# idthanm/env_build

Hardware: AMD Instinct MI355X
Metric: env-steps/s (batched rollout) at N_env x N_veh; achieved HBM GB/s vs peak (higher is better)
Workload: dtype f32

## Files before the change

env_build_amd/csrc/eb_rollout.hip:

```cpp
#include <type_traits>

#include "eb_device.h"
#include "eb_kernels.h"

#pragma clang fp contract(off)

namespace eb {

typedef float f2u __attribute__((ext_vector_type(2), aligned(4)));
typedef float v2f __attribute__((ext_vector_type(2)));
EB_DEV v2f fma2(v2f a, v2f b, v2f c) { return __builtin_elementwise_fma(a, b, c); }

template <typename ST> struct Stored;
template <> struct Stored<float> {
    static EB_DEV f4u load4(const float* p) { return *reinterpret_cast<const f4u*>(p); }
    static EB_DEV float load1(const float* p) { return *p; }
    static EB_DEV void store4(float* p, f4u v) { *reinterpret_cast<f4u*>(p) = v; }
    static EB_DEV void store1(float* p, float v) { *p = v; }
    static EB_DEV float round(float v) { return v; }
    static EB_DEV void store4_wt(float* p, f4u v) { asm volatile("global_store_dwordx4 %0, %1, off sc1\n\ts_nop 1" :: "v"(p), "v"(v) : "memory"); }
    static EB_DEV void store1_wt(float* p, float v) { asm volatile("global_store_dword %0, %1, off sc1" :: "v"(p), "v"(v) : "memory"); }
};
typedef _Float16 h4u __attribute__((ext_vector_type(4), aligned(2)));
template <> struct Stored<_Float16> {
    static EB_DEV f4u load4(const _Float16* p) {
        const h4u h = *reinterpret_cast<const h4u*>(p);
        return f4u{(float)h.x, (float)h.y, (float)h.z, (float)h.w};
    }
    static EB_DEV float load1(const _Float16* p) { return (float)*p; }
    static EB_DEV void store4(_Float16* p, f4u v) {
        *reinterpret_cast<h4u*>(p) = h4u{(_Float16)v.x, (_Float16)v.y, (_Float16)v.z, (_Float16)v.w};
    }
    static EB_DEV void store1(_Float16* p, float v) { *p = (_Float16)v; }
    static EB_DEV float round(float v) { return (float)(_Float16)v; }
    static EB_DEV void store4_wt(_Float16* p, f4u v) {
        typedef unsigned u2v __attribute__((ext_vector_type(2)));
        const u2v bits = __builtin_bit_cast(u2v, h4u{(_Float16)v.x, (_Float16)v.y, (_Float16)v.z, (_Float16)v.w});
        asm volatile("global_store_dwordx2 %0, %1, off sc1" :: "v"(p), "v"(bits) : "memory");
    }
    static EB_DEV void store1_wt(_Float16* p, float v) {
        const unsigned bits = __builtin_bit_cast(unsigned short, (_Float16)v);
        asm volatile("global_store_short %0, %1, off sc1" :: "v"(p), "v"(bits) : "memory");
    }
};

EB_DEV void lds_barrier() { asm volatile("s_waitcnt lgkmcnt(0)\n\ts_barrier" ::: "memory"); }
typedef __attribute__((address_space(3))) int lds_int;
EB_DEV void lds_publish(int* flag, int value) {
    asm volatile("s_waitcnt lgkmcnt(0)" ::: "memory");
    *(volatile lds_int*)flag = value;
}
EB_DEV void lds_wait_until(int* flag, int value) {
    while (*(volatile lds_int*)flag != value) __builtin_amdgcn_s_sleep(2);
    asm volatile("" ::: "memory");
}

template <int CTRL, int ROW_MASK>
EB_DEV double dpp_f64(double v) {
    const unsigned long long b = __builtin_bit_cast(unsigned long long, v);
    const unsigned lo = (unsigned)__builtin_amdgcn_update_dpp(0, (int)(unsigned)b, CTRL, ROW_MASK, 0xf, false);
    const unsigned hi = (unsigned)__builtin_amdgcn_update_dpp(0, (int)(unsigned)(b >> 32), CTRL, ROW_MASK, 0xf, false);
    return __builtin_bit_cast(double, ((unsigned long long)hi << 32) | lo);
}
EB_DEV double wave_sum_f64(double v) {
    v += dpp_f64<0x111, 0xf>(v);
    v += dpp_f64<0x112, 0xf>(v);
    v += dpp_f64<0x114, 0xf>(v);
    v += dpp_f64<0x118, 0xf>(v);
    v += dpp_f64<0x142, 0xa>(v);
    v += dpp_f64<0x143, 0xc>(v);
    return v;
}
template <int CTRL, int ROW_MASK>
EB_DEV float dpp_max_f32(float v) {
    const float o = __builtin_bit_cast(float, __builtin_amdgcn_update_dpp(0, __builtin_bit_cast(int, v), CTRL, ROW_MASK, 0xf, false));
    return o > v ? o : v;
}
EB_DEV float wave_max_f32(float v) {
    v = dpp_max_f32<0x111, 0xf>(v);
    v = dpp_max_f32<0x112, 0xf>(v);
    v = dpp_max_f32<0x114, 0xf>(v);
    v = dpp_max_f32<0x118, 0xf>(v);
    v = dpp_max_f32<0x142, 0xa>(v);
    v = dpp_max_f32<0x143, 0xc>(v);
    return v;
}

EB_DEV void acc_record(double* recs, bool act, int lane, float v_r, float v_t, float v_p) {
    const double s_r = wave_sum_f64(act ? (double)v_r : 0.0);
    const double s_t = wave_sum_f64(act ? (double)v_t : 0.0);
    const double s_p = wave_sum_f64(act ? (double)v_p : 0.0);
    const unsigned long long any = __builtin_amdgcn_ballot_w64(act && v_p > 0.0f);
    if (lane == 63) {
        typedef double d2v __attribute__((ext_vector_type(2)));
        d2v* rec = reinterpret_cast<d2v*>(recs + (size_t)ACC_RECORD_DOUBLES * blockIdx.x);
        rec[0] = d2v{s_r, s_t};
        rec[1] = d2v{s_p, __builtin_bit_cast(double, any)};
    }
}

EB_DEV unsigned agent_load_u32(const unsigned* p) {
    unsigned v;
    asm volatile("global_load_dword %0, %1, off sc1\n\ts_waitcnt vmcnt(0)" : "=v"(v) : "v"(p) : "memory");
    return v;
}
EB_DEV unsigned long long agent_load_u64(const void* p) {
    unsigned long long v;
    asm volatile("global_load_dwordx2 %0, %1, off sc1\n\ts_waitcnt vmcnt(0)" : "=v"(v) : "v"(p) : "memory");
    return v;
}
EB_DEV void agent_store_u32(unsigned* p, unsigned v) { asm volatile("global_store_dword %0, %1, off sc1" :: "v"(p), "v"(v) : "memory"); }
EB_DEV void agent_add_u32(unsigned* p, unsigned v) { asm volatile("global_atomic_add %0, %1, off sc1" :: "v"(p), "v"(v) : "memory"); }

template <typename ST>
struct FusedHot {
    const ST* obs_in;
    ST* obs_out;
    int n_env, obs_dim, n_veh, envs_per_tile;
    unsigned nv_magic;
    int do_rewards;
    double* acc_rec;
    const unsigned char* turn;
    long long t_entry;
};
constexpr int HOT_REWARDS = 1, HOT_PRIO = 2;

template <typename ST>
EB_DEV int env_of_item(const FusedHot<ST>& H, int item) {
    return H.nv_magic ? (int)__umulhi((unsigned)item, H.nv_magic) : item;
}

#define EB_MARK(A, row, i) do { if ((A).trace && (threadIdx.x & 63) == 0) (A).trace[(size_t)(row) * 8 + (i)] = wall_clock64(); } while (0)
#define EB_MARK_PLACE(A, row) do { if ((A).trace && (threadIdx.x & 63) == 0) (A).trace[(size_t)(row) * 8 + 7] = \
    ((long long)__builtin_amdgcn_s_getreg((31 << 11) | 20) << 32) | (unsigned)__builtin_amdgcn_s_getreg((31 << 11) | 4); } while (0)

constexpr int QCAP = 160;
constexpr int TAPE_QCAP = 192;

template <int PRE = 3, bool COARSE = true>
EB_DEV int closest_cell_index(const FusedArgs& A, const float* xy10, const float* phi10, int p, int roff, float px, float py,
                              float& rx, float& ry, float& rphi) {
    const float* xy = xy10 + 2 * roff;
    const float* ph = phi10 + roff;
    const float fx = (px - A.gx0) * CELL_INV, fy = (py - A.gy0) * CELL_INV;
    unsigned c = 0xffffffffu;
    if (fx >= 0.0f && fx < (float)A.gnx && fy >= 0.0f && fy < (float)A.gny) c = A.cells[(p * A.gny + (int)fy) * A.gnx + (int)fx];
    if (c == 0xffffffffu) {
        int r_first = 0, r_last = 1 << 30;
        if constexpr (COARSE) {
            const PathTables& pt = *A.dt;
            int lo, hi, lo2, hi2;
            const int how = coarse_cell_ranges(pt, p, px, py, lo, hi, lo2, hi2);
            if (how == 1) return closest_in_ranges(xy, ph, lo, hi, lo2, hi2, px, py, rx, ry, rphi);
            if (how == 2) { r_first = lo; r_last = hi; }
        }
        const int n = p == 0 ? A.red_len[0] : p == 1 ? A.red_len[1] : A.red_len[2];
        const int bi = closest_reduced_index(reinterpret_cast<const float2*>(xy), A.rad_all + 32 * p, n, px, py, r_first, r_last);
        rx = xy[2 * bi]; ry = xy[2 * bi + 1]; rphi = ph[bi];
        return bi;
    }
    if (PRE > 0 && A.scan_one_trip) return closest_in_range<0>(xy, ph, (int)(c & 0xffffu), (int)(c >> 16), px, py, rx, ry, rphi);
    return closest_in_range<PRE>(xy, ph, (int)(c & 0xffffu), (int)(c >> 16), px, py, rx, ry, rphi);
}

template <int RW, int RPT>
struct FusedSmem {
    static constexpr int ITEMS = RW * 64 * RPT;
    float4 ego[64];
    unsigned char turn[64];
    unsigned long long mask[64];
    float2 pen[ITEMS];
    v2f qxy[RW][QCAP];
    v2f qsc[RW][QCAP];
    int qitem[RW][QCAP];
    int ego_ready;
    int waves_done;
};

template <int TASK, int RW, int RPT, typename ST>
EB_DEV void env_wave(const FusedHot<ST>& H, const FusedArgs& A, FusedSmem<RW, RPT>& S, int e0, int nE) {
    const int lane = threadIdx.x;
    const int D = H.obs_dim, NV = H.n_veh;
    const bool act = lane < nE;
    const int e = act ? lane : 0, ge = e0 + e;
    const ST* hin = H.obs_in + (size_t)ge * D;
    ST* hout = H.obs_out + (size_t)ge * D;

    const f4u h0 = Stored<ST>::load4(hin), h1 = Stored<ST>::load4(hin + 4);
    const float h8 = Stored<ST>::load1(hin + 8);
    const f2u araw = *reinterpret_cast<const f2u*>(A.actions + 2 * (size_t)ge);
    int p = A.path_id;
    if (A.training) {
        const int pr = A.ref_idx[ge];
        p = (pr >= 0 && pr < A.n_paths) ? pr : -1;
    }
    float sh_prev = 0.0f;
    if (A.shield_punish && !A.shield_first && act) sh_prev = A.shield_punish[ge];
    const int trow = blockIdx.x * (RW + 1);
    if (lane == 0) { S.ego_ready = 0; S.waves_done = 0; }
    lds_barrier();
    EB_MARK(A, trow, 0);
    EB_MARK_PLACE(A, trow);
    const bool do_rewards = (H.do_rewards & HOT_REWARDS) != 0;
    const float st[6] = {h0.x, h0.y, h0.z, h0.w, h1.x, h1.y};
    const float phi_rad = deg2rad(st[5]);
    float es, ec;
    sincos_det(phi_rad, es, ec);
    if (do_rewards) {
        S.ego[lane] = make_float4(st[3], st[4], es, ec);
        S.mask[lane] = 0ull;
        lds_publish(&S.ego_ready, 1);
        EB_MARK(A, trow, 1);
    }

    float steer, a_x;
    if (A.actions_raw) action_transform(araw.x, araw.y, steer, a_x);
    else { steer = araw.x; a_x = araw.y; }
    if (act && A.scaled_actions) *reinterpret_cast<f2u*>(A.scaled_actions + 2 * (size_t)ge) = f2u{steer, a_x};
    float rew = 0.0f;
    if (act && do_rewards) {
        const float punish_steer = -sq(steer), punish_a_x = -sq(a_x);
        const float punish_yaw_rate = -sq(st[2]);
        const float devi_y = -sq(h1.z);
        const float devi_phi = -sq(deg2rad(h1.w));
        const float devi_v = -sq(h8);
        rew = 0.05f * devi_v + 0.8f * devi_y + 30.0f * devi_phi + 0.02f * punish_yaw_rate +
              5.0f * punish_steer + 0.05f * punish_a_x;
        A.out5[ge] = rew;
    }
    float nx[6];
    f_xu_core(st, steer, a_x, TAU10, phi_rad, es, ec, nx);
    nx[0] = __builtin_fminf(__builtin_fmaxf(nx[0], 0.0f), 35.0f);
    float t0 = 0.0f, t1 = 0.0f, t2 = 0.0f;
    if (p >= 0) {
        const int roff = p == 0 ? A.red_off[0] : p == 1 ? A.red_off[1] : A.red_off[2];
        EB_MARK(A, trow, 2);
        float rx = 0.0f, ry = 0.0f, rphi = 0.0f;
        constexpr int SCAN_PRE = RW * RPT >= 32 ? 0 : 3;
        const int bi = closest_cell_index<SCAN_PRE>(A, A.xy10, A.phi10, p, roff, nx[3], nx[4], rx, ry, rphi);
        t0 = two2one<TASK>(nx[3], nx[4], rx, ry);
        if (A.trace) { asm volatile("" :: "v"(t0)); EB_MARK(A, trow, 3); }
        t1 = deal_with_phi_diff(nx[5] - rphi);
        t2 = nx[0] - EXP_V;
        if (A.n_future > 0 && act) {
            const PathTables& pt = *A.dt;
            const int len = pt.len[p];
            ST* otrk = hout + 9;
            int cur = bi * 10;
            for (int k = 0; k < A.n_future; ++k) {
                cur += 80;
                if (cur >= len - 2) cur = len - 2;
                const int fi = clamp_index(cur, len);
                Stored<ST>::store1(otrk + 3 * k, pt.x[p][fi] - nx[3]);
                Stored<ST>::store1(otrk + 3 * k + 1, pt.y[p][fi] - nx[4]);
                Stored<ST>::store1(otrk + 3 * k + 2, deal_with_phi_diff(nx[5] - pt.phi[p][fi]));
            }
        }
    } else if (A.n_future > 0 && act) {
        ST* otrk = hout + 9;
        for (int c = 0; c < 3 * A.n_future; ++c) Stored<ST>::store1(otrk + c, 0.0f);
    }
    if (act) {
        Stored<ST>::store4(hout, f4u{nx[0], nx[1], nx[2], nx[3]});
        Stored<ST>::store4(hout + 4, f4u{nx[4], nx[5], t0, t1});
        Stored<ST>::store1(hout + 8, t2);
    }
    EB_MARK(A, trow, 4);
    if (!do_rewards) return;
    float road_t = 0.0f, road_r = 0.0f;
    road_terms<TASK>(st[3] + LWS * ec, st[4] + LWS * es, road_t, road_r);
    road_terms<TASK>(st[3] - LWS * ec, st[4] - LWS * es, road_t, road_r);
    lds_wait_until(&S.waves_done, RW);
    EB_MARK(A, trow, 5);

    float pun_t = 0.0f, pun_r = 0.0f;
    if (act) {
        float a35 = 0.0f, a25 = 0.0f;
        unsigned long long m = S.mask[lane];
        while (m) {
            const int jj = __ffsll((long long)m) - 1;
            m &= m - 1;
            const float2 ps = S.pen[lane * NV + jj];
            a35 += ps.x;
            a25 += ps.y;
        }
        const size_t n = (size_t)H.n_env;
        pun_t = a35 + road_t;
        pun_r = a25 + road_r;
        A.out5[n + ge] = pun_t;
        A.out5[2 * n + ge] = pun_r;
        A.out5[3 * n + ge] = a25;
        A.out5[4 * n + ge] = road_r;
        if (A.shield_punish) {
            const float pacc = sh_prev + (A.shield_row == 3 ? a25 : pun_r);
            A.shield_punish[ge] = pacc;
            if (A.shield_last) A.shield_safe[ge] = pacc > 0.0f ? 0 : 1;
        }
    }
    if (H.acc_rec && A.acc_final) {
        acc_record(H.acc_rec, act, lane, rew, pun_t, pun_r);
        const float dy = __builtin_fabsf(Stored<ST>::round(t0));
        const double s_dy = wave_sum_f64(act ? (double)dy : 0.0);
        const float m_dy = wave_max_f32(act && dy > 0.0f ? dy : 0.0f);
        if (lane == 63) {
            typedef double d2v __attribute__((ext_vector_type(2)));
            reinterpret_cast<d2v*>(A.acc_final)[blockIdx.x] = d2v{s_dy, (double)m_dy};
        }
    }
    EB_MARK(A, trow, 6);
}

template <typename SM, typename ST>
EB_DEV void queue_terms(const FusedHot<ST>& H, SM& S, const float4* ego, int item, float x, float y, float vs, float vc) {
    const int e2 = env_of_item(H, item), j2 = item - e2 * H.n_veh;
    const float4 eg = ego[e2];
    float t35[4], t25[4];
    const float4 pts = make_float4(eg.x + LWS * eg.w, eg.y + LWS * eg.z, eg.x - LWS * eg.w, eg.y - LWS * eg.z);
    veh2veh_terms(pts, x, y, vs, vc, t35, t25);
    const float p35 = ((t35[0] + t35[1]) + t35[2]) + t35[3];
    const float p25 = ((t25[0] + t25[1]) + t25[2]) + t25[3];
    if (p35 != 0.0f) {
        S.pen[item] = make_float2(p35, p25);
        atomicOr(&S.mask[e2], 1ull << j2);
    }
}
template <typename SM, typename ST>
EB_DEV void queue_pass(const FusedHot<ST>& H, SM& S, const float4* ego, int w, int lane, int base, int n) {
    if (lane < n) {
        const v2f vxy = S.qxy[w][base + lane];
        float vs, vc;
        sincos_det(deg2rad(S.qphi[w][base + lane]), vs, vc);
        queue_terms(H, S, ego, S.qitem[w][base + lane], vxy.x, vxy.y, vs, vc);
    }
}
template <typename SM, typename ST>
EB_DEV void queue_pass_sc(const FusedHot<ST>& H, SM& S, const float4* ego, int w, int lane, int base, int n) {
    if (lane < n) {
        const v2f vxy = S.qxy[w][base + lane], sc = S.qsc[w][base + lane];
        queue_terms(H, S, ego, S.qitem[w][base + lane], vxy.x, vxy.y, sc.x, sc.y);
    }
}


template <int TASK, int RW, int RPT, bool FAST, int PF, typename ST>
EB_DEV void record_wave(const FusedHot<ST>& H, const FusedArgs& A, FusedSmem<RW, RPT>& S, int e0, int nE) {
    constexpr int RL = RW * 64;
    const int rtid = threadIdx.x - 64, w = rtid >> 6, lane = rtid & 63;
    const int NV = H.n_veh, D = H.obs_dim, HD = D - 4 * NV;
    const int items = nE * NV;
    const ST* tin = H.obs_in + (size_t)e0 * D;
    ST* tout = H.obs_out + (size_t)e0 * D;
    const int e_first = env_of_item(H, rtid), j_first = rtid - e_first * NV;
    const int epk = RL / NV;
    const int off_first = 4 * rtid + (e_first + 1) * HD, off_step = 4 * RL + epk * HD;
    auto item_of = [&](int k) { return k * RL + rtid; };
    auto env_of = [&](int k) { return FAST ? e_first + k * epk : env_of_item(H, item_of(k)); };
    auto off_of = [&](int k) { return FAST ? off_first + k * off_step : 4 * item_of(k) + (env_of(k) + 1) * HD; };

    static_assert(PF >= 1 && PF <= RPT, "record loads in flight per lane");
    const int turn_code = H.turn[lane];
    f4u rec[PF];
    const bool full_tile = items == RL * RPT;
    auto load_records = [&](auto full_tag) {
        constexpr bool FULL = decltype(full_tag)::value;
#pragma unroll
        for (int k = 0; k < PF; ++k) {
            const bool valid = FULL || item_of(k) < items;
            rec[k] = Stored<ST>::load4(tin + (valid ? off_of(k) : 4 * (items - 1) + nE * HD));
            if (!valid) rec[k].x = 1e30f;
        }
    };
    if (full_tile) load_records(std::true_type{}); else load_records(std::false_type{});
    const bool acc_prev = w == 0 && H.acc_rec && A.prev_out5;
    float pv_r = 0.0f, pv_t = 0.0f, pv_p = 0.0f;
    if (acc_prev && lane < nE) {
        const size_t n = (size_t)H.n_env;
        const float* po = A.prev_out5 + e0 + lane;
        pv_r = po[0]; pv_t = po[n]; pv_p = po[2 * n];
    }
    const int trow = blockIdx.x * (RW + 1) + 1 + w;
    lds_barrier();
    EB_MARK(A, trow, 0);
    EB_MARK_PLACE(A, trow);
    if (A.trace && lane == 0) A.trace[(size_t)trow * 8 + 6] = H.t_entry;
    const bool do_rewards = (H.do_rewards & HOT_REWARDS) != 0;
    const bool by_progress = (H.do_rewards & HOT_PRIO) != 0;
    S.turn[lane] = (unsigned char)turn_code;
    const TurnC tc_lane = turn_consts(S.turn[FAST ? j_first : 0]);
    const SinCosK SK = sincos_consts();

    int qn = 0;
    auto drain = [&]() {
        for (int base = 0; base < qn; base += 64) queue_pass_sc(H, S, S.ego, w, lane, base, min(64, qn - base));
        qn = 0;
    };
    auto near_test = [&](int item, const v2f eg, const f4u r, const v2f sc) {
        const v2f d = v2f{r.x, r.y} - eg;
        const v2f d2 = d * d;
        const bool near = d2.x + d2.y < 40.5f;
        const unsigned long long b = __builtin_amdgcn_ballot_w64(near);
        if (b) {
            if (near) {
                const int pos = (int)__builtin_amdgcn_mbcnt_hi((unsigned)(b >> 32), __builtin_amdgcn_mbcnt_lo((unsigned)b, (unsigned)qn));
                S.qxy[w][pos] = v2f{r.x, r.y};
                S.qsc[w][pos] = sc;
                S.qitem[w][pos] = item;
            }
            qn += __popcll(b);
        }
    };
    if (do_rewards) {
        lds_wait_until(&S.ego_ready, 1);
        EB_MARK(A, trow, 3);
    }
    const bool test_near = do_rewards;
    int k_late = test_near ? RPT : 0;
    auto main_loop = [&](auto full_tag) {
        constexpr bool FULL = decltype(full_tag)::value;
        v2f egoxy[RPT];
        if (test_near) {
#pragma unroll
            for (int k = 0; k < RPT; ++k) {
                const int item = k * RL + rtid;
                const int env = FAST ? e_first + k * epk : env_of_item(H, item);
                egoxy[k] = *reinterpret_cast<const v2f*>(&S.ego[(FULL || item < items) ? env : 0]);
            }
        }
#pragma unroll
        for (int k = 0; k < RPT; ++k) {
            int k_item = k * RL, k_env = k * epk, k_off = k * off_step;
            asm volatile("" : "+s"(k_item), "+s"(k_env), "+s"(k_off));
            const int item = k_item + rtid;
            const int env = FAST ? e_first + k_env : env_of_item(H, item);
            const int off = FAST ? off_first + k_off : 4 * item + (env + 1) * HD;
            const bool valid = FULL || item < items;
            const TurnC tc = FAST ? tc_lane : turn_consts(S.turn[valid ? item - env * NV : 0]);
            float sn, cs;
            if ((k * 4) % RPT == 0 && by_progress)
                switch (3 - (k * 4) / RPT) {
                    case 3: __builtin_amdgcn_s_setprio(3); break;
                    case 2: __builtin_amdgcn_s_setprio(2); break;
                    case 1: __builtin_amdgcn_s_setprio(1); break;
                    default: __builtin_amdgcn_s_setprio(0); break;
                }
            const f4u nv = predict_record_tc<ST>(rec[k % PF], tc, SK, sn, cs);
            if (k < k_late) {
                near_test(item, egoxy[k], rec[k % PF], v2f{sn, cs});
                if (qn > QCAP - 64) k_late = k + 1;
            }
            if (k + PF < RPT) {
                const bool v2 = FULL || item_of(k + PF) < items;
                rec[k % PF] = Stored<ST>::load4(tin + (v2 ? off_of(k + PF) : 4 * (items - 1) + nE * HD));
                if (!v2) rec[k % PF].x = 1e30f;
            }
            if (valid) Stored<ST>::store4(reinterpret_cast<ST*>(reinterpret_cast<char*>(tout) + (unsigned)off * (unsigned)sizeof(ST)), nv);
            if (k == 0) EB_MARK(A, trow, 1);
            if (k == RPT - 1) EB_MARK(A, trow, 2);
            if (k & 1) __builtin_amdgcn_sched_barrier(0);
        }
    };
    if (full_tile) main_loop(std::true_type{}); else main_loop(std::false_type{});
    if (!do_rewards) return;
    if (by_progress) __builtin_amdgcn_s_setprio(0);
    if (test_near && k_late < RPT) {
        for (int k = k_late; k < RPT; ++k) {
            drain();
            const bool valid = item_of(k) < items;
            f4u r = Stored<ST>::load4(tin + (valid ? off_of(k) : 4 * (items - 1) + nE * HD));
            if (!valid) r.x = 1e30f;
            float sn, cs;
            sincos_det(deg2rad(r.w), sn, cs);
            near_test(item_of(k), *reinterpret_cast<const v2f*>(&S.ego[valid ? env_of(k) : 0]), r, v2f{sn, cs});
        }
    }
    EB_MARK(A, trow, 4);
    drain();
    asm volatile("s_waitcnt lgkmcnt(0)" ::: "memory");
    if (lane == 0) atomicAdd(&S.waves_done, 1);
    if (acc_prev) {
        asm volatile("" : "+v"(pv_r), "+v"(pv_t), "+v"(pv_p));
        acc_record(A.prev_rec, lane < nE, lane, pv_r, pv_t, pv_p);
    }
    EB_MARK(A, trow, 5);
}

template <int RW, int RPT>
struct TapeSmem {
    static constexpr int ITEMS = RW * 64 * RPT;
    float4 ego[2][64];
    unsigned char turn[64];
    unsigned long long mask[64];
    float2 pen[ITEMS];
    v2f qxy[RW][TAPE_QCAP];
    float qphi[RW][TAPE_QCAP];
    int qitem[RW][TAPE_QCAP];
    int ego_ready;
    int waves_done;
    int pub_done;
    int abort;
};
EB_DEV bool lds_wait_or_abort(int* flag, int value, int* abort) {
    while (*(volatile lds_int*)flag < value) {
        if (*(volatile lds_int*)abort) return false;
        __builtin_amdgcn_s_sleep(2);
    }
    asm volatile("" ::: "memory");
    return true;
}

struct GateSmem {
    f2u act[2][64];
    float out5[2][5][64];
    float head[2][9][64];
    int bi[2][64];
    int act_ready;
    int out_ready;
    int sent;
};

template <typename ST, bool WT>
EB_DEV void store_head_row(const FusedArgs& A, ST* row, const float (&hv)[9], int bi, int p) {
    auto s4 = [&](ST* q, f4u v) { if (WT) Stored<ST>::store4_wt(q, v); else Stored<ST>::store4(q, v); };
    auto s1 = [&](ST* q, float v) { if (WT) Stored<ST>::store1_wt(q, v); else Stored<ST>::store1(q, v); };
    s4(row, f4u{hv[0], hv[1], hv[2], hv[3]});
    s4(row + 4, f4u{hv[4], hv[5], hv[6], hv[7]});
    s1(row + 8, hv[8]);
    ST* otrk = row + 9;
    if (p >= 0) {
        const PathTables& pt = *A.dt;
        const int len = pt.len[p];
        int cur = bi * 10;
        for (int k = 0; k < A.n_future; ++k) {
            cur += 80;
            if (cur >= len - 2) cur = len - 2;
            const int fi = clamp_index(cur, len);
            s1(otrk + 3 * k, pt.x[p][fi] - hv[3]);
            s1(otrk + 3 * k + 1, pt.y[p][fi] - hv[4]);
            s1(otrk + 3 * k + 2, deal_with_phi_diff(hv[5] - pt.phi[p][fi]));
        }
    } else {
        for (int c = 0; c < 3 * A.n_future; ++c) s1(otrk + c, 0.0f);
    }
}

EB_DEV int env_path(const FusedArgs& A, int ge) {
    if (!A.training) return A.path_id;
    const int pr = A.ref_idx[ge];
    return (pr >= 0 && pr < A.n_paths) ? pr : -1;
}

template <int RW, int RPT>
EB_DEV void in_courier(const FusedArgs& A, TapeSmem<RW, RPT>& S, GateSmem& G, int e0, int nE, int n_env, int horizon) {
    const int lane = threadIdx.x & 63;
    const int ge = e0 + (lane < nE ? lane : 0);
    for (int t = 0; t < horizon; ++t) {
        if (t >= 2 && !lds_wait_or_abort(&G.out_ready, t - 1, &S.abort)) return;
        unsigned open = agent_load_u32(A.gate_ready + t);
        if (!open && t >= 1 && !lds_wait_or_abort(&G.out_ready, t, &S.abort)) return;
        for (int spins = 0; !open && spins <= A.gate_spin; ++spins) {
            open = agent_load_u32(A.gate_ready + t);
            if (open || *(volatile lds_int*)&S.abort) break;
            __builtin_amdgcn_s_sleep(4);
        }
        if (!open) {
            if (lane == 0) agent_store_u32(A.gate_status, 1u);
            lds_publish(&S.abort, 1);
            return;
        }
        const unsigned long long bits = agent_load_u64(A.actions + 2 * ((size_t)t * n_env + ge));
        G.act[t & 1][lane] = __builtin_bit_cast(f2u, bits);
        lds_publish(&G.act_ready, t + 1);
    }
}

template <int RW, int RPT, typename ST>
EB_DEV void out_courier(const FusedHot<ST>& H, const FusedArgs& A, TapeSmem<RW, RPT>& S, GateSmem& G, int e0, int nE, int horizon) {
    const int lane = threadIdx.x & 63;
    const bool act = lane < nE;
    const int ge = e0 + (act ? lane : 0);
    const size_t n = (size_t)H.n_env;
    const int p = env_path(A, ge);
    for (int t = 0; t < horizon; ++t) {
        if (!lds_wait_or_abort(&G.out_ready, t + 1, &S.abort)) return;
        if (act) {
            float* out5 = A.out5 + (size_t)t * 5 * n + ge;
#pragma unroll
            for (int c = 0; c < 5; ++c) Stored<float>::store1_wt(out5 + c * n, G.out5[t & 1][c][lane]);
            if (A.gate_obs) {
                float hv[9];
#pragma unroll
                for (int c = 0; c < 9; ++c) hv[c] = G.head[t & 1][c][lane];
                store_head_row<ST, true>(A, reinterpret_cast<ST*>(A.gate_obs) + ((size_t)t * n + ge) * H.obs_dim, hv, G.bi[t & 1][lane], p);
            }
        }
        asm volatile("s_waitcnt vmcnt(0)" ::: "memory");
        if (A.gate_obs && !lds_wait_or_abort(&S.pub_done, RW * (t + 1), &S.abort)) return;
        if (lane < 4) {
            typedef unsigned u4w __attribute__((ext_vector_type(4)));
            const u4w ones = {1u, 1u, 1u, 1u};
            unsigned* rec = A.gate_done + ((size_t)t * gridDim.x + blockIdx.x) * 16 + 4 * lane;
            asm volatile("global_store_dwordx4 %0, %1, off sc1\n\ts_nop 1" :: "v"(rec), "v"(ones) : "memory");
        }
        lds_publish(&G.sent, t + 1);
    }
}

template <int TASK, int RW, int RPT, bool GATED, typename ST>
EB_DEV void env_wave_tape(const FusedHot<ST>& H, const FusedArgs& A, TapeSmem<RW, RPT>& S, GateSmem* Gp, int e0, int nE, int horizon,
                          const float* xy10, const float* phi10) {
    const int lane = threadIdx.x;
    const int D = H.obs_dim, NV = H.n_veh;
    const bool act = lane < nE;
    const int e = act ? lane : 0, ge = e0 + e;
    const ST* hin = H.obs_in + (size_t)ge * D;
    ST* hout = H.obs_out + (size_t)ge * D;
    const f4u h0 = Stored<ST>::load4(hin), h1 = Stored<ST>::load4(hin + 4);
    float st[6] = {h0.x, h0.y, h0.z, h0.w, h1.x, h1.y};
    float trk[3] = {h1.z, h1.w, Stored<ST>::load1(hin + 8)};
    const int p = env_path(A, ge);
    const int roff = p == 1 ? A.red_off[1] : p == 2 ? A.red_off[2] : A.red_off[0];
    const size_t n = (size_t)H.n_env;
    constexpr bool gated = GATED;
    f2u araw = f2u{0.0f, 0.0f};
    if (!gated) araw = *reinterpret_cast<const f2u*>(A.actions + 2 * (size_t)ge);
    const int trow = blockIdx.x * (RW + 1);
    long long waited = 0;
    EB_MARK(A, trow, 0);
    for (int t = 0; t < horizon; ++t) {
        float* out5 = A.out5 + (size_t)t * 5 * n;
        f2u araw_next = araw;
        if (gated) {
            if (!lds_wait_or_abort(&Gp->act_ready, t + 1, &S.abort)) return;
            araw = Gp->act[t & 1][lane];
            if (t >= 2 && !lds_wait_or_abort(&Gp->sent, t - 1, &S.abort)) return;
        } else if (t + 1 < horizon) {
            araw_next = *reinterpret_cast<const f2u*>(A.actions + 2 * ((size_t)(t + 1) * n + ge));
        }
        const float phi_rad = deg2rad(st[5]);
        float es, ec;
        sincos_det(phi_rad, es, ec);
        S.ego[t & 1][lane] = make_float4(st[3], st[4], es, ec);
        S.mask[lane] = 0ull;
        lds_publish(&S.ego_ready, t + 1);
        float steer, a_x;
        action_transform(araw.x, araw.y, steer, a_x);
        auto put = [&](int c, float v) { if (gated) Gp->out5[t & 1][c][lane] = v; else out5[(size_t)c * n + ge] = v; };
        if (act) {
            const float punish_steer = -sq(steer), punish_a_x = -sq(a_x);
            const float punish_yaw_rate = -sq(st[2]);
            const float devi_y = -sq(trk[0]);
            const float devi_phi = -sq(deg2rad(trk[1]));
            const float devi_v = -sq(trk[2]);
            put(0, 0.05f * devi_v + 0.8f * devi_y + 30.0f * devi_phi + 0.02f * punish_yaw_rate +
                   5.0f * punish_steer + 0.05f * punish_a_x);
        }
        float nx[6];
        f_xu_core(st, steer, a_x, TAU10, phi_rad, es, ec, nx);
        nx[0] = __builtin_fminf(__builtin_fmaxf(nx[0], 0.0f), 35.0f);
        float t0 = 0.0f, t1 = 0.0f, t2 = 0.0f;
        int bi = 0;
        if (p >= 0) {
            float rx = 0.0f, ry = 0.0f, rphi = 0.0f;
            bi = closest_cell_index<0, false>(A, xy10, phi10, p, roff, nx[3], nx[4], rx, ry, rphi);
            t0 = two2one<TASK>(nx[3], nx[4], rx, ry);
            t1 = deal_with_phi_diff(nx[5] - rphi);
            t2 = nx[0] - EXP_V;
        }
        const float hv[9] = {nx[0], nx[1], nx[2], nx[3], nx[4], nx[5], t0, t1, t2};
        if (t == horizon - 1 && act) store_head_row<ST, false>(A, hout, hv, bi, p);
        if (GATED && A.gate_obs) {
#pragma unroll
            for (int c = 0; c < 9; ++c) Gp->head[t & 1][c][lane] = hv[c];
            Gp->bi[t & 1][lane] = bi;
        }
        float road_t = 0.0f, road_r = 0.0f;
        road_terms<TASK>(st[3] + LWS * ec, st[4] + LWS * es, road_t, road_r);
        road_terms<TASK>(st[3] - LWS * ec, st[4] - LWS * es, road_t, road_r);
        const long long w0 = A.trace ? wall_clock64() : 0;
        if (GATED) { if (!lds_wait_or_abort(&S.waves_done, RW * (t + 1), &S.abort)) return; }
        else lds_wait_until(&S.waves_done, RW * (t + 1));
        if (A.trace) waited += wall_clock64() - w0;
        if (act) {
            float a35 = 0.0f, a25 = 0.0f;
            unsigned long long m = S.mask[lane];
            while (m) {
                const int jj = __ffsll((long long)m) - 1;
                m &= m - 1;
                const float2 ps = S.pen[lane * NV + jj];
                a35 += ps.x;
                a25 += ps.y;
            }
            put(1, a35 + road_t);
            put(2, a25 + road_r);
            put(3, a25);
            put(4, road_r);
        }
        if (gated) lds_publish(&Gp->out_ready, t + 1);
#pragma unroll
        for (int c = 0; c < 6; ++c) st[c] = Stored<ST>::round(nx[c]);
        trk[0] = Stored<ST>::round(t0); trk[1] = Stored<ST>::round(t1); trk[2] = Stored<ST>::round(t2);
        araw = araw_next;
    }
    EB_MARK(A, trow, 1);
    if (A.trace && lane == 0) A.trace[(size_t)trow * 8 + 2] = waited;
}

template <int TASK, int RW, int RPT, bool FAST, bool GATED, typename ST>
EB_DEV void record_wave_tape(const FusedHot<ST>& H, const FusedArgs& A, TapeSmem<RW, RPT>& S, int e0, int nE, int horizon) {
    constexpr int RL = RW * 64;
    const int rtid = threadIdx.x - 64, w = rtid >> 6, lane = rtid & 63;
    const int NV = H.n_veh, D = H.obs_dim, HD = D - 4 * NV;
    const int items = nE * NV;
    const ST* tin = H.obs_in + (size_t)e0 * D;
    ST* tout = H.obs_out + (size_t)e0 * D;
    const int e_first = env_of_item(H, rtid), j_first = rtid - e_first * NV;
    const int epk = RL / NV;
    const int off_first = 4 * rtid + (e_first + 1) * HD, off_step = 4 * RL + epk * HD;
    auto item_of = [&](int k) { return k * RL + rtid; };
    auto env_of = [&](int k) { return FAST ? e_first + k * epk : env_of_item(H, item_of(k)); };
    auto off_of = [&](int k) { return FAST ? off_first + k * off_step : 4 * item_of(k) + (env_of(k) + 1) * HD; };
    const int turn_code = A.dt->turn[lane];
    f4u rec[RPT];
#pragma unroll
    for (int k = 0; k < RPT; ++k) {
        const bool valid = item_of(k) < items;
        rec[k] = Stored<ST>::load4(tin + (valid ? off_of(k) : 4 * (items - 1) + nE * HD));
        if (!valid) rec[k].x = 1e30f;
    }
    S.turn[lane] = (unsigned char)turn_code;
    const TurnC tc_lane = turn_consts(S.turn[FAST ? j_first : 0]);
    const SinCosK SK = sincos_consts();
    const int trow = blockIdx.x * (RW + 1) + 1 + w;
    long long waited = 0;
    EB_MARK(A, trow, 0);
    for (int t = 0; t < horizon; ++t) {
        const float4* ego = S.ego[t & 1];
        int qn = 0;
        auto drain = [&]() {
            for (int base = 0; base < qn; base += 64) queue_pass(H, S, ego, w, lane, base, min(64, qn - base));
            qn = 0;
        };
        const long long w0 = A.trace ? wall_clock64() : 0;
        if (GATED) { if (!lds_wait_or_abort(&S.ego_ready, t + 1, &S.abort)) return; }
        else lds_wait_until(&S.ego_ready, t + 1);
        if (A.trace) waited += wall_clock64() - w0;
#pragma unroll
        for (int k = 0; k < RPT; ++k) {
            int k_item = k * RL, k_env = k * epk;
            asm volatile("" : "+s"(k_item), "+s"(k_env));
            const int item = k_item + rtid;
            const int env = FAST ? e_first + k_env : env_of_item(H, item);
            if (k > 0 && (k & 1) == 0 && qn > 64) drain();
            const float4 eg = ego[item < items ? env : 0];
            const v2f d = v2f{rec[k].x, rec[k].y} - v2f{eg.x, eg.y};
            const v2f d2 = d * d;
            const bool near = d2.x + d2.y < 40.5f;
            const unsigned long long b = __builtin_amdgcn_ballot_w64(near);
            if (b) {
                if (near) {
                    const int pos = (int)__builtin_amdgcn_mbcnt_hi((unsigned)(b >> 32), __builtin_amdgcn_mbcnt_lo((unsigned)b, (unsigned)qn));
                    S.qxy[w][pos] = v2f{rec[k].x, rec[k].y};
                    S.qphi[w][pos] = rec[k].w;
                    S.qitem[w][pos] = item;
                }
                qn += __popcll(b);
            }
        }
        drain();
        asm volatile("s_waitcnt lgkmcnt(0)" ::: "memory");
        if (lane == 0) atomicAdd(&S.waves_done, 1);
#pragma unroll
        for (int k = 0; k < RPT; ++k) {
            int k_item = k * RL, k_env = k * epk;
            asm volatile("" : "+s"(k_item), "+s"(k_env));
            const int item = k_item + rtid;
            if (item < items) {
                const int env = FAST ? e_first + k_env : env_of_item(H, item);
                const TurnC tc = FAST ? tc_lane : turn_consts(S.turn[item - env * NV]);
                float sn_, cs_;
                const f4u nv = predict_record_tc<ST>(rec[k], tc, SK, sn_, cs_);
                rec[k] = f4u{Stored<ST>::round(nv.x), Stored<ST>::round(nv.y), Stored<ST>::round(nv.z), Stored<ST>::round(nv.w)};
                if (GATED && A.gate_obs) Stored<ST>::store4_wt(reinterpret_cast<ST*>(A.gate_obs) + ((size_t)t * H.n_env + e0) * D + off_of(k), rec[k]);
            }
            if (k & 1) __builtin_amdgcn_sched_barrier(0);
        }
        if (GATED && A.gate_obs) {
            asm volatile("s_waitcnt vmcnt(0)" ::: "memory");
            if (lane == 0) atomicAdd(&S.pub_done, 1);
        }
    }
#pragma unroll
    for (int k = 0; k < RPT; ++k)
        if (item_of(k) < items) Stored<ST>::store4(tout + off_of(k), rec[k]);
    EB_MARK(A, trow, 1);
    if (A.trace && lane == 0) A.trace[(size_t)trow * 8 + 2] = waited;
}

template <int TASK, int RW, int RPT, bool FAST, bool GATED, typename ST>
EB_DEV void tape_body(const FusedHot<ST>& H, const FusedArgs& A, int horizon) {
    __shared__ TapeSmem<RW, RPT> S;
    extern __shared__ __attribute__((aligned(16))) float staged[];
    const int e0 = blockIdx.x * H.envs_per_tile;
    const int nE = min(H.envs_per_tile, H.n_env - e0);
    __shared__ std::conditional_t<GATED, GateSmem, int> Gs;
    GateSmem* Gp = GATED ? reinterpret_cast<GateSmem*>(&Gs) : nullptr;
    if (threadIdx.x == 0) {
        S.ego_ready = 0; S.waves_done = 0; S.pub_done = 0; S.abort = 0;
        if (GATED) { Gp->act_ready = 0; Gp->out_ready = 0; Gp->sent = 0; }
    }
    const float* xy10 = A.xy10;
    const float* phi10 = A.phi10;
    if (A.stage_entries > 0) {
        const int n_xy = 2 * A.stage_entries, n_all = 3 * A.stage_entries;
        for (int i = threadIdx.x; i < n_all; i += (RW + (GATED ? 3 : 1)) * 64) staged[i] = i < n_xy ? A.xy10[i] : A.phi10[i - n_xy];
        xy10 = staged;
        phi10 = staged + n_xy;
    }
    lds_barrier();
    if (threadIdx.x < 64) {
        __builtin_amdgcn_s_setprio(3);
        env_wave_tape<TASK, RW, RPT, GATED, ST>(H, A, S, Gp, e0, nE, horizon, xy10, phi10);
    }
    else if (threadIdx.x < (RW + 1) * 64) record_wave_tape<TASK, RW, RPT, FAST, GATED, ST>(H, A, S, e0, nE, horizon);
    else if (GATED && threadIdx.x < (RW + 2) * 64) in_courier<RW, RPT>(A, S, *Gp, e0, nE, H.n_env, horizon);
    else if (GATED) out_courier<RW, RPT, ST>(H, A, S, *Gp, e0, nE, horizon);
}

template <int TASK, int RW, int RPT, bool FAST, int PF, typename ST>
EB_DEV void fused_body(const FusedHot<ST>& H, const FusedArgs& A) {
    __shared__ FusedSmem<RW, RPT> S;
    const int e0 = blockIdx.x * H.envs_per_tile;
    const int nE = min(H.envs_per_tile, H.n_env - e0);
    if (RW * RPT >= 32) asm volatile("; keep v79 allocated" ::: "v79");
    if (threadIdx.x < 64) {
        __builtin_amdgcn_s_setprio(2);
        env_wave<TASK, RW, RPT, ST>(H, A, S, e0, nE);
    } else {
        record_wave<TASK, RW, RPT, FAST, PF, ST>(H, A, S, e0, nE);
    }
}

#define EB_FUSED_KERNEL(NAME, RW, RPT, WAVES, VGPRS)                                                     \
    template <int TASK, bool FAST, int PF, typename ST>                                                  \
    __global__ __launch_bounds__((RW + 1) * 64, WAVES) __attribute__((amdgpu_num_vgpr(VGPRS))) void NAME( \
        const ST* obs_in, ST* obs_out, int n_env, int obs_dim, int n_veh, int envs_per_tile,             \
        unsigned nv_magic, int do_rewards, double* acc_rec, const unsigned char* turn_tab, const FusedArgs A) { \
        const FusedHot<ST> H{obs_in, obs_out, n_env, obs_dim, n_veh, envs_per_tile, nv_magic, do_rewards, acc_rec, turn_tab, \
                             wall_clock64()};                                                            \
        fused_body<TASK, RW, RPT, FAST, PF, ST>(H, A);                                                   \
    }
EB_FUSED_KERNEL(rollout_fused_4x8, 4, 8, 6, 80)
EB_FUSED_KERNEL(rollout_fused_4x4, 4, 4, 6, 80)
EB_FUSED_KERNEL(rollout_fused_1x4, 1, 4, 6, 80)

#define EB_TAPE_KERNEL(NAME, RW, RPT, GATED, WAVES)                                                      \
    template <int TASK, bool FAST, typename ST>                                                          \
    __global__ __launch_bounds__((RW + (GATED ? 3 : 1)) * 64, WAVES) void NAME(                          \
        const ST* obs_in, ST* obs_out, int n_env, int obs_dim, int n_veh, int envs_per_tile,             \
        unsigned nv_magic, int horizon, const FusedArgs A) {                                             \
        const FusedHot<ST> H{obs_in, obs_out, n_env, obs_dim, n_veh, envs_per_tile, nv_magic, HOT_REWARDS, nullptr, nullptr, 0ll}; \
        tape_body<TASK, RW, RPT, FAST, GATED, ST>(H, A, horizon);                                        \
    }
EB_TAPE_KERNEL(rollout_tape_4x8, 4, 8, false, 6)
EB_TAPE_KERNEL(rollout_tape_4x4, 4, 4, false, 1)
EB_TAPE_KERNEL(rollout_tape_1x4, 1, 4, false, 1)
EB_TAPE_KERNEL(rollout_gated_4x8, 4, 8, true, 4)
EB_TAPE_KERNEL(rollout_gated_4x4, 4, 4, true, 1)
EB_TAPE_KERNEL(rollout_gated_1x4, 1, 4, true, 1)

int tape_tile_variant(int variant, int n_veh, int storage_f16) {
    (void)storage_f16;
    return (variant == 0 && (4 * 64) % n_veh != 0) ? 1 : variant;
}

int fused_tile_records(int variant) {
    switch (variant) {
        case 0: return 4 * 64 * 8;
        case 1: return 4 * 64 * 4;
        default: return 1 * 64 * 4;
    }
}

int tape_blocks_per_cu(int task, int variant, int n_veh, int storage_f16, size_t dyn_bytes) {
    (void)task;
    const int rw = variant == 0 || variant == 1 ? 4 : 1;
    int nb = 0;
    const hipError_t e = with_bool(storage_f16, [&](auto f16) { return with_bool((rw * 64) % n_veh == 0, [&](auto fast) {
        using ST = std::conditional_t<f16, _Float16, float>;
        auto occ = [&](auto kernel) { return hipOccupancyMaxActiveBlocksPerMultiprocessor(&nb, kernel, (rw + 3) * 64, dyn_bytes); };
        return variant == 0 ? occ(rollout_gated_4x8<TASK_LEFT, fast, ST>) : variant == 1 ? occ(rollout_gated_4x4<TASK_LEFT, fast, ST>)
                                                                          : occ(rollout_gated_1x4<TASK_LEFT, fast, ST>);
    }); });
    return e == hipSuccess ? nb : 0;
}

typedef unsigned u4v __attribute__((ext_vector_type(4)));
__global__ __launch_bounds__(256) void gate_feed_kernel(int horizon, unsigned n_blocks, size_t step_words, const u4v* __restrict__ staged,
                                                        u4v* live, unsigned* gate_ready, const unsigned* gate_done,
                                                        unsigned* status, int spin) {
    constexpr int PRE = 8;
    for (int t = 0; t < horizon; ++t) {
        const u4v* src = staged + (size_t)t * step_words;
        u4v* dst = live + (size_t)t * step_words;
        u4v pre[PRE];
#pragma unroll
        for (int k = 0; k < PRE; ++k) {
            const size_t i = threadIdx.x + (size_t)k * blockDim.x;
            pre[k] = src[i < step_words ? i : 0];
        }
        int good = 1;
        if (t > 0) {
            for (unsigned b = threadIdx.x; b < n_blocks && good; b += blockDim.x) {
                const unsigned* w = gate_done + ((size_t)(t - 1) * n_blocks + b) * 16;
                for (int spins = 0; !agent_load_u32(w); ++spins) {
                    if (spins >= spin || ((spins & 31) == 31 && agent_load_u32(status))) { good = 0; break; }
                    __builtin_amdgcn_s_sleep(2);
                }
            }
        }
        if (!__syncthreads_and(good)) {
            if (threadIdx.x == 0) agent_store_u32(status + 1, 1u);
            return;
        }
#pragma unroll
        for (int k = 0; k < PRE; ++k) {
            const size_t i = threadIdx.x + (size_t)k * blockDim.x;
            if (i < step_words) asm volatile("global_store_dwordx4 %0, %1, off sc1\n\ts_nop 1" :: "v"(dst + i), "v"(pre[k]) : "memory");
        }
        for (size_t i = threadIdx.x + (size_t)PRE * blockDim.x; i < step_words; i += blockDim.x) {
            const u4v v = src[i];
            asm volatile("global_store_dwordx4 %0, %1, off sc1\n\ts_nop 1" :: "v"(dst + i), "v"(v) : "memory");
        }
        asm volatile("s_waitcnt vmcnt(0)" ::: "memory");
        __syncthreads();
        if (threadIdx.x == 0) agent_store_u32(gate_ready + t, 1u);
    }
}

hipError_t launch_gate_feed(int horizon, int n_blocks, size_t step_bytes, const void* staged, void* live,
                            unsigned* gate_ready, const unsigned* gate_done, unsigned* status, int spin, hipStream_t s) {
    hipLaunchKernelGGL(gate_feed_kernel, dim3(1), dim3(256), 0, s, horizon, (unsigned)n_blocks, step_bytes / 16,
                       reinterpret_cast<const u4v*>(staged), reinterpret_cast<u4v*>(live), gate_ready, gate_done, status, spin);
    return hipGetLastError();
}

static FusedArgs trace_checked(const FusedArgs& A_in, int grid, int waves_per_block) {
    FusedArgs A = A_in;
    if (A.trace && A.trace_words < (long long)grid * waves_per_block * 8) A.trace = nullptr;
    return A;
}

hipError_t launch_rollout_tape_fused(int task, int variant, const FusedArgs& A_in, int horizon, int grid, hipStream_t s) {
    const int rw = variant == 0 || variant == 1 ? 4 : 1;
    const FusedArgs A = trace_checked(A_in, grid, rw + 1);
    const bool gated = A.gate_ready != nullptr, fast = (rw * 64) % A.n_veh == 0;
    if (variant == 0 && !gated && !fast) return hipErrorInvalidValue;
    const dim3 g(grid), b((rw + 1 + (gated ? 2 : 0)) * 64);
    const size_t dyn = (size_t)A.stage_entries * 12;
    with_task(task, [&](auto t) { with_bool(A.storage_f16, [&](auto f16) { with_bool(fast, [&](auto fast_c) {
        using ST = std::conditional_t<f16, _Float16, float>;
        auto go = [&](auto kernel) {
            hipLaunchKernelGGL(kernel, g, b, dyn, s, reinterpret_cast<const ST*>(A.obs_in), reinterpret_cast<ST*>(A.obs_out), A.n_env,
                               A.obs_dim, A.n_veh, A.envs_per_tile, A.nv_magic, horizon, A);
        };
        if (gated && variant == 0) go(rollout_gated_4x8<t, fast_c, ST>);
        else if (gated && variant == 1) go(rollout_gated_4x4<t, fast_c, ST>);
        else if (gated) go(rollout_gated_1x4<t, fast_c, ST>);
        else if (variant == 0) go(rollout_tape_4x8<t, true, ST>);
        else if (variant == 1) go(rollout_tape_4x4<t, fast_c, ST>);
        else go(rollout_tape_1x4<t, fast_c, ST>);
    }); }); });
    return hipGetLastError();
}

hipError_t launch_rollout_fused(int task, int variant, const FusedArgs& A_in, int grid, hipStream_t s) {
    const int rw = variant == 0 || variant == 1 ? 4 : 1;
    const FusedArgs A = trace_checked(A_in, grid, rw + 1);
    const dim3 g(grid), b((rw + 1) * 64);
    const int hot = (A.do_rewards ? HOT_REWARDS : 0) | (A.by_progress ? HOT_PRIO : 0);
    const unsigned char* turn_tab = reinterpret_cast<const unsigned char*>(A.dt) + offsetof(PathTables, turn);
    with_task(task, [&](auto t) { with_bool(A.storage_f16, [&](auto f16) { with_bool((rw * 64) % A.n_veh == 0, [&](auto fast) {
        using ST = std::conditional_t<f16, _Float16, float>;
        auto go = [&](auto kernel) {
            hipLaunchKernelGGL(kernel, g, b, 0, s, reinterpret_cast<const ST*>(A.obs_in), reinterpret_cast<ST*>(A.obs_out), A.n_env,
                               A.obs_dim, A.n_veh, A.envs_per_tile, A.nv_magic, hot, A.acc_rec, turn_tab, A);
        };
        if (variant == 0 && A.rolling) go(rollout_fused_4x8<t, fast, 3, ST>);
        else if (variant == 0) go(rollout_fused_4x8<t, fast, 8, ST>);
        else if (variant == 1) go(rollout_fused_4x4<t, fast, 4, ST>);
        else go(rollout_fused_1x4<t, fast, 4, ST>);
    }); }); });
    return hipGetLastError();
}

}
```

Measured before the change: 4.330 billion.

## Offload near-pair penalty queue draining from record waves to the env wave

Record waves now publish their near-pair queue counts progressively through per-wave LDS counters instead of draining the queues themselves. The env wave, which previously just waited for all record waves to finish, consumes published queue entries in 64-wide batches and computes the vehicle-vehicle penalty terms. The aim is to move the penalty work onto an otherwise idle wave and off the record waves' critical path. Overflow items are now evaluated inline, and the record prediction is rewritten with precomputed reciprocal constants. This adds LDS polling and publish traffic, and depends on correct ordering between producer and consumer through the queue.

Measured after the change: 4.255 billion. -1.7%, worse.

```diff
diff --git a/env_build_amd/csrc/eb_rollout.hip b/env_build_amd/csrc/eb_rollout.hip
--- a/env_build_amd/csrc/eb_rollout.hip
+++ b/env_build_amd/csrc/eb_rollout.hip
@@ -175,7 +175,46 @@
     int qitem[RW][QCAP];
     int ego_ready;
     int waves_done;
+    int q_pub[RW];
 };
+
+template <typename SM, typename ST>
+EB_DEV void queue_terms(const FusedHot<ST>& H, SM& S, const float4* ego, int item, float x, float y, float vs, float vc);
+
+template <int RW, int RPT, typename ST>
+EB_DEV void drain_queues(const FusedHot<ST>& H, FusedSmem<RW, RPT>& S, int lane) {
+    int cons[RW];
+#pragma unroll
+    for (int w = 0; w < RW; ++w) cons[w] = 0;
+    for (;;) {
+        const int done = __builtin_amdgcn_readfirstlane(*(volatile lds_int*)&S.waves_done);
+        int pub[RW], avail = 0;
+#pragma unroll
+        for (int w = 0; w < RW; ++w) {
+            pub[w] = __builtin_amdgcn_readfirstlane(*(volatile lds_int*)&S.q_pub[w]);
+            avail += pub[w] - cons[w];
+        }
+        asm volatile("" ::: "memory");
+        if (avail >= 64 || (done == RW && avail > 0)) {
+            int slot = -1, start = 0, left = 64;
+#pragma unroll
+            for (int w = 0; w < RW; ++w) {
+                const int a = pub[w] - cons[w], i = lane - start;
+                if (i >= 0 && i < a) slot = w * QCAP + cons[w] + i;
+                const int t = min(a, left);
+                start += a; cons[w] += t; left -= t;
+            }
+            if (slot >= 0) {
+                const v2f vxy = (&S.qxy[0][0])[slot], sc = (&S.qsc[0][0])[slot];
+                queue_terms(H, S, S.ego, (&S.qitem[0][0])[slot], vxy.x, vxy.y, sc.x, sc.y);
+            }
+        } else if (done == RW) {
+            break;
+        } else {
+            __builtin_amdgcn_s_sleep(2);
+        }
+    }
+}
 
 template <int TASK, int RW, int RPT, typename ST>
 EB_DEV void env_wave(const FusedHot<ST>& H, const FusedArgs& A, FusedSmem<RW, RPT>& S, int e0, int nE) {
@@ -198,6 +237,7 @@
     if (A.shield_punish && !A.shield_first && act) sh_prev = A.shield_punish[ge];
     const int trow = blockIdx.x * (RW + 1);
     if (lane == 0) { S.ego_ready = 0; S.waves_done = 0; }
+    if (lane < RW) S.q_pub[lane] = 0;
     lds_barrier();
     EB_MARK(A, trow, 0);
     EB_MARK_PLACE(A, trow);
@@ -270,7 +310,7 @@
     float road_t = 0.0f, road_r = 0.0f;
     road_terms<TASK>(st[3] + LWS * ec, st[4] + LWS * es, road_t, road_r);
     road_terms<TASK>(st[3] - LWS * ec, st[4] - LWS * es, road_t, road_r);
-    lds_wait_until(&S.waves_done, RW);
+    drain_queues(H, S, lane);
     EB_MARK(A, trow, 5);
 
     float pun_t = 0.0f, pun_r = 0.0f;
@@ -333,14 +373,33 @@
         queue_terms(H, S, ego, S.qitem[w][base + lane], vxy.x, vxy.y, vs, vc);
     }
 }
-template <typename SM, typename ST>
-EB_DEV void queue_pass_sc(const FusedHot<ST>& H, SM& S, const float4* ego, int w, int lane, int base, int n) {
-    if (lane < n) {
-        const v2f vxy = S.qxy[w][base + lane], sc = S.qsc[w][base + lane];
-        queue_terms(H, S, ego, S.qitem[w][base + lane], vxy.x, vxy.y, sc.x, sc.y);
-    }
-}
-
+
+
+struct PredictK { double r10, r180, rpi; };
+EB_DEV PredictK predict_consts() {
+    PredictK k{1.0 / (double)C10::value, 1.0 / (double)C180::value, 1.0 / (double)CPi::value};
+    asm volatile("" : "+s"(k.r10), "+s"(k.r180), "+s"(k.rpi));
+    return k;
+}
+EB_DEV f4u predict_record_k(const f4u rec, const TurnC tc, const SinCosK K, const PredictK P, float& sn_out, float& cs_out) {
+    const float v = rec.z;
+    const float v10 = div_by(v, P.r10);
+    const float phi_rad = div_by(rec.w * PI_F, P.r180);
+    float sn, cs;
+    sincos_det_k(phi_rad, K, sn, cs);
+    sn_out = sn; cs_out = cs;
+    const float nx_ = rec.x + v10 * cs, ny_ = rec.y + v10 * sn;
+    const bool middle = (rec.x > -HALF_CROSS && rec.x < HALF_CROSS) && (rec.y > -HALF_CROSS && rec.y < HALF_CROSS);
+    const float u = div_by(v, tc.rc);
+    const float u10 = div_by(u, P.r10);
+    const bool turning = middle && tc.enabled != 0.0f;
+    const float dphi = turning ? u10 : 0.0f;
+    float nphi = phi_rad + dphi;
+    if (nphi > PI_F) nphi = nphi - TWO_PI_F;
+    if (nphi <= -PI_F) nphi = nphi + TWO_PI_F;
+    const float nphi_deg = div_by(nphi * 180.0f, P.rpi);
+    return f4u{nx_, ny_, v, nphi_deg};
+}
 
 template <int TASK, int RW, int RPT, bool FAST, int PF, typename ST>
 EB_DEV void record_wave(const FusedHot<ST>& H, const FusedArgs& A, FusedSmem<RW, RPT>& S, int e0, int nE) {
@@ -388,12 +447,9 @@
     S.turn[lane] = (unsigned char)turn_code;
     const TurnC tc_lane = turn_consts(S.turn[FAST ? j_first : 0]);
     const SinCosK SK = sincos_consts();
+    const PredictK PK = predict_consts();
 
     int qn = 0;
-    auto drain = [&]() {
-        for (int base = 0; base < qn; base += 64) queue_pass_sc(H, S, S.ego, w, lane, base, min(64, qn - base));
-        qn = 0;
-    };
     auto near_test = [&](int item, const v2f eg, const f4u r, const v2f sc) {
         const v2f d = v2f{r.x, r.y} - eg;
         const v2f d2 = d * d;
@@ -443,7 +499,8 @@
                     case 1: __builtin_amdgcn_s_setprio(1); break;
                     default: __builtin_amdgcn_s_setprio(0); break;
                 }
-            const f4u nv = predict_record_tc<ST>(rec[k % PF], tc, SK, sn, cs);
+            const f4u nv = predict_record_k(rec[k % PF], tc, SK, PK, sn, cs);
+            if (test_near && k >= 2 && (k & 1) == 0) lds_publish(&S.q_pub[w], qn);
             if (k < k_late) {
                 near_test(item, egoxy[k], rec[k % PF], v2f{sn, cs});
                 if (qn > QCAP - 64) k_late = k + 1;
@@ -462,19 +519,22 @@
     if (full_tile) main_loop(std::true_type{}); else main_loop(std::false_type{});
     if (!do_rewards) return;
     if (by_progress) __builtin_amdgcn_s_setprio(0);
+    lds_publish(&S.q_pub[w], qn);
     if (test_near && k_late < RPT) {
         for (int k = k_late; k < RPT; ++k) {
-            drain();
             const bool valid = item_of(k) < items;
             f4u r = Stored<ST>::load4(tin + (valid ? off_of(k) : 4 * (items - 1) + nE * HD));
             if (!valid) r.x = 1e30f;
-            float sn, cs;
-            sincos_det(deg2rad(r.w), sn, cs);
-            near_test(item_of(k), *reinterpret_cast<const v2f*>(&S.ego[valid ? env_of(k) : 0]), r, v2f{sn, cs});
+            const v2f d = v2f{r.x, r.y} - *reinterpret_cast<const v2f*>(&S.ego[valid ? env_of(k) : 0]);
+            const v2f d2 = d * d;
+            if (d2.x + d2.y < 40.5f) {
+                float sn, cs;
+                sincos_det(deg2rad(r.w), sn, cs);
+                queue_terms(H, S, S.ego, item_of(k), r.x, r.y, sn, cs);
+            }
         }
     }
     EB_MARK(A, trow, 4);
-    drain();
     asm volatile("s_waitcnt lgkmcnt(0)" ::: "memory");
     if (lane == 0) atomicAdd(&S.waves_done, 1);
     if (acc_prev) {
```
